# hank-kuo-cs/Volumetric-Primitives-Net

Measured on AMD Instinct MI355X. Metric: render+Chamfer fwd+bwd images/sec, higher is better.
Workload: dtype f32; 1 GPU; C3: B=64/GPU (global 64), K=32 sphere primitives, 256x256 silhouette+depth, n=256 pts/prim (N=8192) vs M=2048 GT points, Chamfer+L1 fwd+bwd; global_batch=64, parallelism=dp1, collective=none, sampling=fresh Philox draws every step (device step counter, 28 steps drawn)

## Files before the change

### volumetric-primitives-net_amd/csrc/sampler.hip

```cpp
#include "vpn_raster_common.h"
#include "vpn_chamfer_feat.h"

namespace vpn {

constexpr int SAMP_BLOCK = 256;

struct PrimLds {
    Pose pose;
    float v[3];
    int cum[7];
    int kind;
};

__device__ inline void cuboid_quota(const float v[3], int n, int cum[7]) {
#pragma clang fp contract(off)
    float w = v[0], h = v[1], d = v[2];
    float hd = h * d, dw = d * w, wh = w * h;
    float total = (hd + dw + wh) * 2.0f;
    float area[6] = {hd, hd, dw, dw, wh, wh};
    int acc = 0;
    cum[0] = 0;
#pragma unroll
    for (int f = 0; f < 5; ++f) {
        float weight = area[f] / total;
        int c = (int)rintf((float)n * weight);
        acc += c;
        cum[f + 1] = acc;
    }
    cum[6] = n;
}

__device__ inline void canonical_coeff(const PrimLds& P, int p, const float u[3], float c[3]) {
    if (P.kind == VPN_SPHERE) {
        const float w0 = 1.0f - 2.0f * u[0];
        const float ce0 = 2.0f * sqrtf(u[0] * (1.0f - u[0]));
        const float w = fmaf(VPN_HALF_PI_EXCESS, ce0, w0);
        const float ce = fmaf(-VPN_HALF_PI_EXCESS, w0, ce0);
        const float azim = u[1] * 2.0f * VPN_PI;
        float sa, ca;
        sincosf(azim, &sa, &ca);
        c[0] = ce * sa;
        c[1] = w;
        c[2] = ce * ca;
    } else {
        c[0] = -1.0f + 2.0f * u[0];
        c[1] = -1.0f + 2.0f * u[1];
        c[2] = -1.0f + 2.0f * u[2];
#pragma unroll
        for (int f = 0; f < 6; ++f) {
            if (p >= P.cum[f] && p < P.cum[f + 1]) c[f >> 1] = (f & 1) ? -1.0f : 1.0f;
        }
    }
}

__device__ inline void load_prim(PrimLds& P, const float* prm, int kind, int n) {
    P.pose = make_pose(prm[3], prm[4], prm[5], prm[6]);
    P.v[0] = prm[0]; P.v[1] = prm[1]; P.v[2] = prm[2];
    P.kind = kind == VPN_SPHERE ? VPN_SPHERE : VPN_CUBOID;
    if (P.kind == VPN_CUBOID) cuboid_quota(P.v, n, P.cum);
}

__device__ inline void load_prim_saved(PrimLds& P, const float* prm, int kind, int n, const float4* rk) {
    const float4 p0 = rk[R_FIN + 3], p1 = rk[R_FIN + 4], p2 = rk[R_FIN + 5], p3 = rk[R_FIN + 6];
    Pose& S = P.pose;
    S.R.m[0][0] = p0.x; S.R.m[0][1] = p0.y; S.R.m[0][2] = p0.z; S.R.m[1][0] = p0.w; S.R.m[1][1] = p1.x; S.R.m[1][2] = p1.y;
    S.R.m[2][0] = p1.z; S.R.m[2][1] = p1.w; S.R.m[2][2] = p2.x; S.x = p2.y; S.y = p2.z; S.z = p2.w;
    S.w = p3.x; S.sh = p3.y; S.ch = p3.z; S.inv_len = p3.w;
    P.v[0] = prm[0]; P.v[1] = prm[1]; P.v[2] = prm[2];
    P.kind = kind == VPN_SPHERE ? VPN_SPHERE : VPN_CUBOID;
    if (P.kind == VPN_CUBOID) cuboid_quota(P.v, n, P.cum);
}

__device__ inline void sample_wg(PrimLds& P, float* red, int b, int k,
    const float* __restrict__ params, const int32_t* __restrict__ kinds, const float* __restrict__ u,
    uint64_t seed, uint64_t sample_base, int K, int n,
    float* __restrict__ points, const RasterPrep& rp, const FeatJob* feat, const FeatJob* gt = nullptr,
    float* red_gt = nullptr) {
    const float* prm = params + ((size_t)b * K + k) * VPN_PARAM_STRIDE;
    if (threadIdx.x == 0) load_prim(P, prm, kinds[k], n);
    if (gt) feat_slice_early(*gt, b, k, 64, red_gt);
    Camera C;
    const bool rec_lane = rp.rec && threadIdx.x == 64;
    if (rec_lane) C = make_camera(rp.cam + b * 3);
    if (rp.zero_me && k == 0) {
        if (b == 0 && threadIdx.x >= 128 && threadIdx.x < 130) rp.zero_me[threadIdx.x - 128] = 0;
        if (b == 0 && threadIdx.x == 130) *reinterpret_cast<uint64_t*>(rp.zero_me + 2) = seed;
        if (threadIdx.x == 131) rp.zero_me[4 + 4 * b + 3] = 0;
    }
    __syncthreads();
    if (gt && threadIdx.x == 65) feat_slice_publish(*gt, b, k, 64, red_gt);
    if (rec_lane) {
        float4 r[R_REC];
        make_record_from(C, P.pose, prm, kinds[k] == VPN_SPHERE ? VPN_SPHERE : VPN_CUBOID, rp.H, rp.W, rp.sigma, r);
        float4* out = rp.rec + ((size_t)b * K + k) * R_REC;
#pragma unroll
        for (int i = 0; i < R_REC; ++i) out[i] = r[i];
    }
    const float tx = prm[7], ty = prm[8], tz = prm[9];
    const float* ub = u ? u + ((size_t)b * K + k) * n * 3 : nullptr;
    float* out = points + ((size_t)b * K + k) * n * 3;
    float nv = 0.0f;
    for (int p = threadIdx.x; p < n; p += SAMP_BLOCK) {
        float uu[3];
        if (ub) { uu[0] = ub[p * 3]; uu[1] = ub[p * 3 + 1]; uu[2] = ub[p * 3 + 2]; }
        else philox_uniform3(seed, sample_base + (uint64_t)b, (uint32_t)k, (uint32_t)p, uu);
        float c[3];
        canonical_coeff(P, p, uu, c);
        float px, py, pz;
        {
#pragma clang fp contract(off)
            const float x = c[0] * P.v[0], y = c[1] * P.v[1], z = c[2] * P.v[2];
            const Mat3& R = P.pose.R;
            px = (R.m[0][0] * x + R.m[0][1] * y + R.m[0][2] * z) + tx;
            py = (R.m[1][0] * x + R.m[1][1] * y + R.m[1][2] * z) + ty;
            pz = (R.m[2][0] * x + R.m[2][1] * y + R.m[2][2] * z) + tz;
        }
        st3(out + p * 3, px, py, pz);
        if (feat) nv = fmaxf(nv, feat_point(*feat, b, k * n + p, px, py, pz));
    }
    if (feat) {
        if (k == K - 1) for (int j = K * n + (int)threadIdx.x; j < feat->Np; j += SAMP_BLOCK) feat_point(*feat, b, j, 0.f, 0.f, 0.f);
        if (feat->tboxes) __threadfence_block();
        feat_finish_slice(*feat, b, k, nv, red);
        feat_tile_boxes(*feat, b, k * n, k == K - 1 ? feat->Np : (k + 1) * n);
    }
}

__global__ __launch_bounds__(SAMP_BLOCK) void sample_fwd_kernel(
    const float* __restrict__ params, const int32_t* __restrict__ kinds, const float* __restrict__ u,
    uint64_t seed, const uint64_t* __restrict__ seed_dev, uint64_t sample_base, int K, int n,
    float* __restrict__ points, const RasterPrep rp) {
    __shared__ PrimLds P;
    if (seed_dev) seed += *seed_dev;
    sample_wg(P, nullptr, blockIdx.y, blockIdx.x, params, kinds, u, seed, sample_base, K, n, points, rp, nullptr);
}

__host__ __device__ inline int rec_workgroups(int BK) { return ((BK + SAMP_BLOCK - 1) / SAMP_BLOCK + 7) & ~7; }
__host__ __device__ inline int ord_workgroups(int B) { return (B + 7) & ~7; }

__global__ __launch_bounds__(SAMP_BLOCK) void sample_feat_fwd_kernel(
    const float* __restrict__ params, const int32_t* __restrict__ kinds, const float* __restrict__ u,
    uint64_t seed, const uint64_t* __restrict__ seed_dev, uint64_t sample_base, int B, int K, int n,
    float* __restrict__ points, const RasterPrep rp, const FeatJob pred, const FeatJob gt) {
    __shared__ PrimLds P;
    __shared__ float red[SAMP_BLOCK / 64];
    static_assert(SAMP_BLOCK == CFEAT_THREADS, "feature slices are written by sampler-sized workgroups");
    if (seed_dev) seed += *seed_dev;
    const int nrec = rp.rec ? rec_workgroups(B * K) : 0;
    if ((int)blockIdx.x < nrec) {
        const int bk = blockIdx.x * SAMP_BLOCK + threadIdx.x;
        if (bk < B * K) {
            const int rb = bk / K, rk = bk - rb * K;
            const float* prm = params + (size_t)bk * VPN_PARAM_STRIDE;
            const Camera C = make_camera(rp.cam + rb * 3);
            const Pose Pq = make_pose(prm[3], prm[4], prm[5], prm[6]);
            float4* out = rp.rec + (size_t)bk * R_REC;
            make_record_put(C, Pq, prm, kinds[rk] == VPN_SPHERE ? VPN_SPHERE : VPN_CUBOID, rp.H, rp.W, rp.sigma,
                            [&](int i, const float4 v) { out[i] = v; });
        }
        return;
    }
    const int nord = gt.perm ? ord_workgroups(B) : 0;
    if ((int)blockIdx.x < nrec + nord) {
        int ob, oy;
        feat_decode((int)blockIdx.x - nrec, nord, ob, oy);
        if (ob < B) feat_order_wg(gt, ob);
        return;
    }
    RasterPrep rq = rp;
    rq.rec = nullptr;
    int b, sy;
    feat_decode((int)blockIdx.x - nrec - nord, B, b, sy);
    __shared__ float red_gt[SAMP_BLOCK / 64];
    sample_wg(P, red, b, sy, params, kinds, u, seed, sample_base, K, n, points, rq, &pred, &gt, red_gt);
}

__global__ __launch_bounds__(SAMP_BLOCK) void sample_bwd_kernel(
    const float* __restrict__ params, const int32_t* __restrict__ kinds, const float* __restrict__ u,
    uint64_t seed, const uint64_t* __restrict__ seed_dev, uint64_t sample_base, int K, int n,
    const float* __restrict__ grad_points, float* __restrict__ grad_params) {
    __shared__ PrimLds P;
    if (seed_dev) seed += *seed_dev;
    __shared__ float red[SAMP_BLOCK / 64][12];
    const int k = blockIdx.x, b = blockIdx.y;
    const float* prm = params + ((size_t)b * K + k) * VPN_PARAM_STRIDE;
    if (threadIdx.x == 0) load_prim(P, prm, kinds[k], n);
    __syncthreads();
    const float* ub = u ? u + ((size_t)b * K + k) * n * 3 : nullptr;
    const float* gp = grad_points + ((size_t)b * K + k) * n * 3;
    float acc[12];
#pragma unroll
    for (int i = 0; i < 12; ++i) acc[i] = 0.0f;
    for (int p = threadIdx.x; p < n; p += SAMP_BLOCK) {
        float uu[3];
        if (ub) { uu[0] = ub[p * 3]; uu[1] = ub[p * 3 + 1]; uu[2] = ub[p * 3 + 2]; }
        else philox_uniform3(seed, sample_base + (uint64_t)b, (uint32_t)k, (uint32_t)p, uu);
        float c[3];
        canonical_coeff(P, p, uu, c);
        float g[3] = {gp[p * 3], gp[p * 3 + 1], gp[p * 3 + 2]};
#pragma unroll
        for (int r = 0; r < 3; ++r) {
#pragma unroll
            for (int a = 0; a < 3; ++a) acc[r * 3 + a] += g[r] * c[a];
            acc[9 + r] += g[r];
        }
    }
    const int lane = threadIdx.x & 63, wave = threadIdx.x >> 6;
#pragma unroll
    for (int i = 0; i < 12; ++i) {
        float s = wave_sum(acc[i]);
        if (lane == 0) red[wave][i] = s;
    }
    __syncthreads();
    if (threadIdx.x == 0) {
        float G[3][3], gt[3];
        for (int r = 0; r < 3; ++r) {
            for (int a = 0; a < 3; ++a) {
                float s = 0.0f;
                for (int w = 0; w < SAMP_BLOCK / 64; ++w) s += red[w][r * 3 + a];
                G[r][a] = s;
            }
            float s = 0.0f;
            for (int w = 0; w < SAMP_BLOCK / 64; ++w) s += red[w][9 + r];
            gt[r] = s;
        }
        const Mat3& R = P.pose.R;
        float gR[3][3], gv[3], gq[4];
        for (int a = 0; a < 3; ++a) {
            gv[a] = R.m[0][a] * G[0][a] + R.m[1][a] * G[1][a] + R.m[2][a] * G[2][a];
            for (int r = 0; r < 3; ++r) gR[r][a] = G[r][a] * P.v[a];
        }
        pose_backward(P.pose, prm[3], prm[4], prm[5], gR, gq);
        float* o = grad_params + ((size_t)b * K + k) * VPN_PARAM_STRIDE;
        o[0] = gv[0]; o[1] = gv[1]; o[2] = gv[2];
        o[3] = gq[0]; o[4] = gq[1]; o[5] = gq[2]; o[6] = gq[3];
        o[7] = gt[0]; o[8] = gt[1]; o[9] = gt[2];
    }
}

#ifndef SCB_BLOCK
#define SCB_BLOCK 128
#endif
struct StepExtras {
    const float* emd_dist = nullptr; const int32_t* emd_assign = nullptr; float emd_coef = 0.f;
    const float* dv_dist1 = nullptr; const int32_t* dv_idx1 = nullptr;
    const float* dv_dist2 = nullptr; const int32_t* dv_idx2 = nullptr;
    float dv_c1 = 0.f, dv_c2 = 0.f;
    const float* cn_points = nullptr; const float* cn_gt = nullptr; const float* cn_mat = nullptr;
    const float* cn_dist1 = nullptr; const int32_t* cn_idx1 = nullptr; const float* cn_dist2 = nullptr; const int32_t* cn_idx2 = nullptr;
    float cn_c1 = 0.f, cn_c2 = 0.f; int cn_M = 0;
};

template <bool EXTRAS>
__global__ __launch_bounds__(SCB_BLOCK) void sample_chamfer_bwd_kernel(
    const float* __restrict__ params, const int32_t* __restrict__ kinds, const float* __restrict__ u,
    uint64_t seed, const uint64_t* __restrict__ seed_dev, uint64_t sample_base, int K, int n,
    const float* __restrict__ points, const float* __restrict__ gt, int M, const float* __restrict__ dist1, const int32_t* __restrict__ idx1,
    const float* __restrict__ dist2, const int32_t* __restrict__ idx2, const float* __restrict__ grad_loss_b,
    float w1, float w2, float* __restrict__ grad_params, const RasterFinish rf, const StepExtras ex) {
    __shared__ PrimLds P;
    __shared__ float red[SCB_BLOCK / 64][12];
    __shared__ float fin[SCB_BLOCK / 64][12];
    __shared__ float rgrad[10];
    if (seed_dev) seed += *seed_dev;
    const int k = blockIdx.x, b = blockIdx.y, N = K * n;
    const float* prm = params + ((size_t)b * K + k) * VPN_PARAM_STRIDE;
    if (threadIdx.x == 0) {
        if (rf.rec) load_prim_saved(P, prm, kinds[k], n, rf.rec + ((size_t)b * K + k) * R_REC);
        else load_prim(P, prm, kinds[k], n);
    }
    if (rf.partial) {
        float fv[16];
        raster_finish_gather(b * K + k, K, rf.ntile, rf.words, rf.masks, rf.partial, (int)(threadIdx.x >> 6) * 64, SCB_BLOCK, fv);
        const float tot = wave_reduce16_swap(fv);
        if ((threadIdx.x & 3) == 0 && (threadIdx.x & 63) < 48) fin[threadIdx.x >> 6][(threadIdx.x & 63) >> 2] = tot;
    }
    __syncthreads();
    const float* ub = u ? u + ((size_t)b * K + k) * n * 3 : nullptr;
    const float* A = points + (size_t)b * N * 3;
    const float* G2 = gt + (size_t)b * M * 3;
    const float gl = grad_loss_b ? grad_loss_b[b] : rf.scale[0];
    const float ca = gl * w1 / (float)N, cb = gl * w2 / (float)M;
    float acc[12];
#pragma unroll
    for (int i = 0; i < 12; ++i) acc[i] = 0.0f;
    const float tx = prm[7], ty = prm[8], tz = prm[9];
    const float vmin = fminf(fminf(fabsf(P.v[0]), fabsf(P.v[1])), fabsf(P.v[2]));
    const float big = fmaxf(fmaxf(fmaxf(fabsf(tx), fabsf(ty)), fabsf(tz)), fmaxf(fmaxf(fabsf(P.v[0]), fabsf(P.v[1])), fabsf(P.v[2])));
    const bool recover = vmin >= 1.0e-2f * big && vmin > 1e-20f;
    const float iv0 = recover ? 1.0f / P.v[0] : 0.0f, iv1 = recover ? 1.0f / P.v[1] : 0.0f, iv2 = recover ? 1.0f / P.v[2] : 0.0f;
    auto add = [&](int pl, float gx, float gy, float gz) {
        float c[3];
        if (recover) {
            const int i = k * n + pl;
            const F3 a = ld3(A + i * 3);
            const float dx = a.x - tx, dy = a.y - ty, dz = a.z - tz;
            const Mat3& R = P.pose.R;
            c[0] = (R.m[0][0] * dx + R.m[1][0] * dy + R.m[2][0] * dz) * iv0;
            c[1] = (R.m[0][1] * dx + R.m[1][1] * dy + R.m[2][1] * dz) * iv1;
            c[2] = (R.m[0][2] * dx + R.m[1][2] * dy + R.m[2][2] * dz) * iv2;
        } else {
            float uu[3];
            if (ub) { uu[0] = ub[pl * 3]; uu[1] = ub[pl * 3 + 1]; uu[2] = ub[pl * 3 + 2]; }
            else philox_uniform3(seed, sample_base + (uint64_t)b, (uint32_t)k, (uint32_t)pl, uu);
            canonical_coeff(P, pl, uu, c);
        }
        const float g[3] = {gx, gy, gz};
#pragma unroll
        for (int r = 0; r < 3; ++r) {
#pragma unroll
            for (int a = 0; a < 3; ++a) acc[r * 3 + a] += g[r] * c[a];
            acc[9 + r] += g[r];
        }
    };
    const bool cn_on = EXTRAS && ex.cn_points;
    const float* Sm = ex.cn_mat + b * 9;
    const float S0 = cn_on ? Sm[0] : 0.f, S1 = cn_on ? Sm[1] : 0.f, S2 = cn_on ? Sm[2] : 0.f, S3 = cn_on ? Sm[3] : 0.f, S4 = cn_on ? Sm[4] : 0.f,
                S5 = cn_on ? Sm[5] : 0.f, S6 = cn_on ? Sm[6] : 0.f, S7 = cn_on ? Sm[7] : 0.f, S8 = cn_on ? Sm[8] : 0.f;
    auto add_canon = [&](int pl, float gx, float gy, float gz) {
        add(pl, S0 * gx + S3 * gy + S6 * gz, S1 * gx + S4 * gy + S7 * gz, S2 * gx + S5 * gy + S8 * gz);
    };
    for (int pl = threadIdx.x; pl < n; pl += SCB_BLOCK) {
        const int i = k * n + pl, j = idx1[(size_t)b * N + i];
        const float coef = ca / dist1[(size_t)b * N + i];
        const F3 a = ld3(A + i * 3), g = ld3(G2 + j * 3);
        float gx = coef * (a.x - g.x), gy = coef * (a.y - g.y), gz = coef * (a.z - g.z);
        if (EXTRAS && ex.emd_dist) {
// ... 277 lines not shown
                float s = 0.0f;
                for (int w = 0; w < MESH_BLOCK / 64; ++w) s += red[w][r * 3 + a];
                G[r][a] = s;
            }
            float s = 0.0f;
            for (int w = 0; w < MESH_BLOCK / 64; ++w) s += red[w][9 + r];
            gt[r] = s;
        }
        const Mat3& R = S.R;
        float gR[3][3], gv[3], gq[4];
        for (int a = 0; a < 3; ++a) {
            gv[a] = R.m[0][a] * G[0][a] + R.m[1][a] * G[1][a] + R.m[2][a] * G[2][a];
            for (int r = 0; r < 3; ++r) gR[r][a] = G[r][a] * prm[a];
        }
        pose_backward(S, prm[3], prm[4], prm[5], gR, gq);
        float* og = grad_params + ((size_t)b * K + k) * VPN_PARAM_STRIDE;
        og[0] = gv[0]; og[1] = gv[1]; og[2] = gv[2];
        og[3] = gq[0]; og[4] = gq[1]; og[5] = gq[2]; og[6] = gq[3];
        og[7] = gt[0]; og[8] = gt[1]; og[9] = gt[2];
    }
}

__device__ inline Mat3 mat_mul(const Mat3& A, const Mat3& B) {
    Mat3 C;
#pragma unroll
    for (int i = 0; i < 3; ++i)
#pragma unroll
        for (int j = 0; j < 3; ++j) C.m[i][j] = A.m[i][0] * B.m[0][j] + A.m[i][1] * B.m[1][j] + A.m[i][2] * B.m[2][j];
    return C;
}

__device__ inline Mat3 camera_matrix(float elev, float azim, float angle, int to_object) {
    const float e = elev / 360.0f, a = azim / 360.0f;
    const Mat3 Re = make_pose(0.0f, 0.0f, -1.0f, e).R;
    const float yx = Re.m[0][1], yy = Re.m[1][1], yz = Re.m[2][1];
    if (to_object) {
        const Mat3 Rx = make_pose(1.0f, 0.0f, 0.0f, -angle / 360.0f).R;
        const Mat3 Ra = make_pose(yx, yy, yz, -a).R;
        const Mat3 Rb = make_pose(0.0f, 0.0f, -1.0f, -e).R;
        return mat_mul(Rb, mat_mul(Ra, Rx));
    }
    const Mat3 Ra = make_pose(yx, yy, yz, a).R;
    return mat_mul(Ra, Re);
}

__global__ __launch_bounds__(TR_BLOCK) void camera_transform_kernel(
    const float* __restrict__ pts, const float* __restrict__ dists, const float* __restrict__ elevs,
    const float* __restrict__ azims, const float* __restrict__ angles, int N, int to_object, int transpose,
    float* __restrict__ out) {
    __shared__ Mat3 S;
    const int b = blockIdx.y;
    if (threadIdx.x == 0) {
        Mat3 M = camera_matrix(elevs[b], azims[b], angles ? angles[b] : 0.0f, to_object);
        if (transpose) {
            Mat3 T;
            for (int i = 0; i < 3; ++i) for (int j = 0; j < 3; ++j) T.m[i][j] = M.m[j][i];
            M = T;
        }
        S = M;
    }
    __syncthreads();
    const Mat3& R = S;
    const float d = dists[b];
    for (int p = blockIdx.x * TR_BLOCK + threadIdx.x; p < N; p += gridDim.x * TR_BLOCK) {
        const float* pp = pts + ((size_t)b * N + p) * 3;
        const float x = pp[0], y = pp[1], z = pp[2];
        float ox = R.m[0][0] * x + R.m[0][1] * y + R.m[0][2] * z;
        float oy = R.m[1][0] * x + R.m[1][1] * y + R.m[1][2] * z;
        float oz = R.m[2][0] * x + R.m[2][1] * y + R.m[2][2] * z;
        if (to_object) { ox *= d; oy *= d; oz *= d; }
        else { ox /= d; oy /= d; oz /= d; }
        float* o = out + ((size_t)b * N + p) * 3;
        o[0] = ox; o[1] = oy; o[2] = oz;
    }
}

__global__ __launch_bounds__(64) void camera_matrix_kernel(const float* __restrict__ dists, const float* __restrict__ elevs,
                                                          const float* __restrict__ azims, const float* __restrict__ angles,
                                                          int B, int to_object, float* __restrict__ mat) {
    const int b = blockIdx.x * 64 + threadIdx.x;
    if (b >= B) return;
    const Mat3 M = camera_matrix(elevs[b], azims[b], angles ? angles[b] : 0.0f, to_object);
    const float d = dists[b];
    for (int i = 0; i < 3; ++i) for (int j = 0; j < 3; ++j) mat[b * 9 + i * 3 + j] = to_object ? M.m[i][j] * d : M.m[i][j] / d;
}

__global__ __launch_bounds__(256) void raster_prep_kernel(const float* __restrict__ params,
                                                          const int32_t* __restrict__ kinds,
                                                          const float* __restrict__ cam, int BK, int K, int H, int W,
                                                          float sigma, float4* __restrict__ rec, int* __restrict__ zero_me) {
    const int bk = blockIdx.x * 256 + threadIdx.x;
    if (zero_me && bk < 4) zero_me[bk] = 0;
    if (bk >= BK) return;
    const int b = bk / K, k = bk - b * K;
    if (zero_me && k == 0) zero_me[4 + 4 * b + 3] = 0;
    float4 r[R_REC];
    make_record(params + (size_t)bk * VPN_PARAM_STRIDE, kinds[k] == VPN_SPHERE ? VPN_SPHERE : VPN_CUBOID, cam, b, H, W, sigma, r);
    float4* out = rec + (size_t)bk * R_REC;
#pragma unroll
    for (int i = 0; i < R_REC; ++i) out[i] = r[i];
}


int launch_raster_prep(const float* params, const int32_t* kinds, const float* cam, int B, int K, int H, int W,
                       float sigma, void* records, int* zero_me, hipStream_t s) {
    const int BK = B * K;
    VPN_LAUNCH(raster_prep_kernel, dim3((BK + 255) / 256), dim3(256), 0, s, params, kinds, cam, BK, K, H, W, sigma,
               (float4*)records, zero_me);
    VPN_LAUNCH_CHECK();
    return 0;
}

}

using namespace vpn;

static int launch_sample_fwd(const float* params, const int32_t* kinds, const float* u, uint64_t seed,
                             const uint64_t* seed_dev, uint64_t sample_base, int B, int K, int n, float* points,
                             const RasterPrep& rp, void* stream) {
    if (!params || !kinds || !points) return VPN_E_BADARG;
    if (B <= 0 || K <= 0 || n <= 0) return VPN_E_BADARG;
    if (B > 65535) return VPN_E_TOOBIG;
    VPN_LAUNCH(sample_fwd_kernel, dim3(K, B), dim3(SAMP_BLOCK), 0, (hipStream_t)stream, params, kinds, u,
                       seed, seed_dev, sample_base, K, n, points, rp);
    VPN_LAUNCH_CHECK();
    return 0;
}

extern "C" int vpn_sample_fwd(const float* params, const int32_t* kinds, const float* u, uint64_t seed,
                              const uint64_t* seed_dev, uint64_t sample_base, int B, int K, int n, float* points,
                              void* stream) {
    return launch_sample_fwd(params, kinds, u, seed, seed_dev, sample_base, B, K, n, points, RasterPrep{}, stream);
}

extern "C" int vpn_hotpath_sample_fwd(const float* params, const int32_t* kinds, const float* u, uint64_t seed,
                                      const uint64_t* seed_dev, uint64_t sample_base, int B, int K, int n, float* points,
                                      const float* cam, int H, int W, float sigma, void* records, void* loss_ws,
                                      const float* gt_points, int M, void* chamfer_ws, size_t chamfer_ws_bytes,
                                      void* stream) {
    if (!cam || !records || H <= 0 || W <= 0 || !(sigma > 0.f) || K > VPN_MAX_PRIMS) return VPN_E_BADARG;
    if (((uintptr_t)records & 15) != 0) return VPN_E_BADARG;
    RasterPrep rp;
    rp.cam = cam; rp.H = H; rp.W = W; rp.sigma = sigma; rp.rec = (float4*)records; rp.zero_me = (int*)loss_ws;
    if (!chamfer_ws) return launch_sample_fwd(params, kinds, u, seed, seed_dev, sample_base, B, K, n, points, rp, stream);
    if (!params || !kinds || !points || !gt_points) return VPN_E_BADARG;
    if (B <= 0 || K <= 0 || n <= 0 || M <= 0 || K > CFEAT_SLOTS) return VPN_E_BADARG;
    if ((long long)B * K * n > 0x7fffffffLL) return VPN_E_TOOBIG;
    FeatJob pred, gt;
    int rc = chamfer_feat_jobs(chamfer_ws, chamfer_ws_bytes, B, K * n, M, points, gt_points, &pred, &gt);
    if (rc) return rc;
    pred.ysplit = K;
    gt.ysplit = K;
    const unsigned nrec = (unsigned)rec_workgroups(B * K) + (gt.perm ? (unsigned)ord_workgroups(B) : 0u);
    VPN_LAUNCH(sample_feat_fwd_kernel, dim3((unsigned)B * (unsigned)K + nrec), dim3(SAMP_BLOCK), 0, (hipStream_t)stream,
               params, kinds, u, seed, seed_dev, sample_base, B, K, n, points, rp, pred, gt);
    VPN_LAUNCH_CHECK();
    return 0;
}

extern "C" int vpn_hotpath_fused_features(int B, int K, int n, int M) {
    if (B <= 0 || K <= 0 || n <= 0 || M <= 0 || K > CFEAT_SLOTS) return 0;
    FeatJob a, b;
    static float dummy[4] __attribute__((aligned(16)));
    return chamfer_feat_jobs(dummy, (size_t)-1, B, K * n, M, nullptr, nullptr, &a, &b) == 0 ? 1 : 0;
}

extern "C" int vpn_sample_bwd(const float* params, const int32_t* kinds, const float* u, uint64_t seed,
                              const uint64_t* seed_dev, uint64_t sample_base, int B, int K, int n, const float* grad_points,
                              float* grad_params, void* stream) {
    if (!params || !kinds || !grad_points || !grad_params) return VPN_E_BADARG;
    if (B <= 0 || K <= 0 || n <= 0) return VPN_E_BADARG;
    if (B > 65535) return VPN_E_TOOBIG;
    VPN_LAUNCH(sample_bwd_kernel, dim3(K, B), dim3(SAMP_BLOCK), 0, (hipStream_t)stream, params, kinds, u,
                       seed, seed_dev, sample_base, K, n, grad_points, grad_params);
    VPN_LAUNCH_CHECK();
    return 0;
}

extern "C" int vpn_transform_fwd(const float* points, const float* q, const float* t, int B, int N, float* out,
                                 void* stream) {
    if (!points || !q || !out) return VPN_E_BADARG;
    if (B <= 0 || N <= 0) return VPN_E_BADARG;
    if (B > 65535) return VPN_E_TOOBIG;
    int gx = (N + TR_BLOCK - 1) / TR_BLOCK;
    if (gx > 1024) gx = 1024;
    VPN_LAUNCH(transform_fwd_kernel, dim3(gx, B), dim3(TR_BLOCK), 0, (hipStream_t)stream, points, q, t, N,
                       out);
    VPN_LAUNCH_CHECK();
    return 0;
}

extern "C" int vpn_transform_bwd(const float* points, const float* q, const float* grad_out, int B, int N,
                                 float* grad_points, float* grad_q, float* grad_t, void* stream) {
    if (!points || !q || !grad_out) return VPN_E_BADARG;
    if (B <= 0 || N <= 0) return VPN_E_BADARG;
    VPN_LAUNCH(transform_bwd_kernel, dim3(B), dim3(TR_BLOCK), 0, (hipStream_t)stream, points, q, grad_out,
                       N, grad_points, grad_q, grad_t);
    VPN_LAUNCH_CHECK();
    return 0;
}

static int camera_launch(const float* points, const float* dists, const float* elevs, const float* azims,
                         const float* angles, int B, int N, int to_object, int transpose, float* out, void* stream) {
    if (!points || !dists || !elevs || !azims || !out) return VPN_E_BADARG;
    if (to_object && !angles) return VPN_E_BADARG;
    if (B <= 0 || N <= 0) return VPN_E_BADARG;
    if (B > 65535) return VPN_E_TOOBIG;
    int gx = (N + TR_BLOCK - 1) / TR_BLOCK;
    if (gx > 1024) gx = 1024;
    VPN_LAUNCH(camera_transform_kernel, dim3(gx, B), dim3(TR_BLOCK), 0, (hipStream_t)stream, points, dists, elevs,
               azims, angles, N, to_object, transpose, out);
    VPN_LAUNCH_CHECK();
    return 0;
}

extern "C" int vpn_camera_matrix(const float* dists, const float* elevs, const float* azims, const float* angles, int B,
                                 int to_object, float* mat, void* stream) {
    if (!dists || !elevs || !azims || !mat || (to_object && !angles) || B <= 0) return VPN_E_BADARG;
    VPN_LAUNCH(camera_matrix_kernel, dim3((B + 63) / 64), dim3(64), 0, (hipStream_t)stream, dists, elevs, azims, angles, B, to_object, mat);
    VPN_LAUNCH_CHECK();
    return 0;
}

extern "C" int vpn_camera_transform_fwd(const float* points, const float* dists, const float* elevs,
                                        const float* azims, const float* angles, int B, int N, int to_object,
                                        float* out, void* stream) {
    return camera_launch(points, dists, elevs, azims, angles, B, N, to_object, 0, out, stream);
}

extern "C" int vpn_camera_transform_bwd(const float* grad_out, const float* dists, const float* elevs,
                                        const float* azims, const float* angles, int B, int N, int to_object,
                                        float* grad_points, void* stream) {
    return camera_launch(grad_out, dists, elevs, azims, angles, B, N, to_object, 1, grad_points, stream);
}

static constexpr size_t SCB_MAX_LDS = 60 * 1024;
static constexpr size_t scb_match_lds(int M) {
    return (size_t)((M + SCB_BLOCK - 1) / SCB_BLOCK) * 64 * (SCB_BLOCK / 64) * sizeof(int2);
}
static_assert(scb_match_lds(VPN_FUSED_BWD_MAX_GT) <= SCB_MAX_LDS && scb_match_lds(VPN_FUSED_BWD_MAX_GT + 1) > SCB_MAX_LDS,
              "VPN_FUSED_BWD_MAX_GT is the largest M whose match lists fit");

static int launch_scb(const float* params, const int32_t* kinds, const float* u, uint64_t seed,
                      const uint64_t* seed_dev, uint64_t sample_base, int B, int K, int n, const float* points,
                      const float* gt_points, int M, const float* dist1, const int32_t* idx1,
                      const float* dist2, const int32_t* idx2, const float* grad_loss_b, float w1,
                      float w2, float* grad_params, const RasterFinish& rf, void* stream, const StepExtras* ex = nullptr) {
    if (!params || !kinds || !points || !gt_points || !dist1 || !idx1 || !dist2 || !idx2 || !grad_params)
        return VPN_E_BADARG;
    if (!grad_loss_b && !rf.scale) return VPN_E_BADARG;
    if (B <= 0 || K <= 0 || n <= 0 || M <= 0) return VPN_E_BADARG;
    if (B > 65535 || (long long)K * n > 0x7fffffffLL / 3) return VPN_E_TOOBIG;
    constexpr int BLK = SCB_BLOCK;
    const size_t lds = scb_match_lds(M);
    if (lds > SCB_MAX_LDS) return VPN_E_TOOBIG;
    if (ex)
        VPN_LAUNCH_AS("sample_chamfer_bwd_kernel<step>", sample_chamfer_bwd_kernel<true>, dim3(K, B), dim3(BLK), lds, (hipStream_t)stream, params, kinds, u, seed,
                      seed_dev, sample_base, K, n, points, gt_points, M, dist1, idx1, dist2, idx2, grad_loss_b, w1, w2, grad_params, rf, *ex);
    else
        VPN_LAUNCH_AS("sample_chamfer_bwd_kernel", sample_chamfer_bwd_kernel<false>, dim3(K, B), dim3(BLK), lds, (hipStream_t)stream, params, kinds, u, seed,
                      seed_dev, sample_base, K, n, points, gt_points, M, dist1, idx1, dist2, idx2, grad_loss_b, w1, w2, grad_params, rf, StepExtras{});
    VPN_LAUNCH_CHECK();
    return 0;
}

extern "C" int vpn_sample_chamfer_bwd(const float* params, const int32_t* kinds, const float* u, uint64_t seed,
                                      const uint64_t* seed_dev, uint64_t sample_base, int B, int K, int n, const float* points,
                                      const float* gt_points, int M, const float* dist1, const int32_t* idx1,
                                      const float* dist2, const int32_t* idx2, const float* grad_loss_b, float w1,
                                      float w2, float* grad_params, void* stream) {
    return launch_scb(params, kinds, u, seed, seed_dev, sample_base, B, K, n, points, gt_points, M, dist1, idx1, dist2, idx2,
                      grad_loss_b, w1, w2, grad_params, RasterFinish{}, stream);
}

extern "C" int vpn_hotpath_bwd(const float* params, const int32_t* kinds, const float* u, uint64_t seed,
                               const uint64_t* seed_dev, uint64_t sample_base, int B, int K, int n, const float* points,
                               const float* gt_points, int M, const float* dist1, const int32_t* idx1,
                               const float* dist2, const int32_t* idx2, const float* grad_loss_b, float w1, float w2,
                               const float* cam, int H, int W, const void* records, const void* workspace,
                               const float* grad_total, float* grad_params, void* stream) {
    if (!cam || !records || !workspace || H <= 0 || W <= 0) return VPN_E_BADARG;
    RasterFinish rf;
    rf.rec = (const float4*)records;
    rf.ntile = ((W + R_TW - 1) / R_TW) * ((H + R_TH - 1) / R_TH);
    rf.words = (K + 63) / 64;
    rf.masks = reinterpret_cast<const unsigned long long*>(reinterpret_cast<const char*>(records) + (size_t)B * K * R_REC * sizeof(float4));
    rf.partial = (const float*)workspace;
    rf.scale = grad_total;
    return launch_scb(params, kinds, u, seed, seed_dev, sample_base, B, K, n, points, gt_points, M, dist1, idx1, dist2, idx2,
                      grad_loss_b, w1, w2, grad_params, rf, stream);
}

extern "C" int vpn_trainstep_bwd(const float* params, const int32_t* kinds, uint64_t seed, const uint64_t* seed_dev,
                                 uint64_t sample_base, int B, int K, int n, const float* points, const float* gt_points, int M,
                                 const float* dist1, const int32_t* idx1, const float* dist2, const int32_t* idx2,
                                 float w1, float w2, const float* cam, int H, int W, const void* records,
                                 const void* workspace, const float* grad_total,
                                 const float* emd_dist, const int32_t* emd_assign, float emd_coef,
                                 const float* dv_dist1, const int32_t* dv_idx1, const float* dv_dist2, const int32_t* dv_idx2,
                                 float dv_c1, float dv_c2,
                                 const float* cn_points, const float* cn_gt, const float* cn_mat, const float* cn_dist1,
                                 const int32_t* cn_idx1, const float* cn_dist2, const int32_t* cn_idx2, float cn_c1, float cn_c2,
                                 int cn_M, float* grad_params, void* stream) {
    if (!grad_total) return VPN_E_BADARG;
    if (emd_dist && (!emd_assign || K * n != M)) return VPN_E_BADARG;
    if (dv_dist1 && (!dv_idx1 || !dv_dist2 || !dv_idx2)) return VPN_E_BADARG;
    if (cn_points && (!cn_gt || !cn_mat || !cn_dist1 || !cn_idx1 || !cn_dist2 || !cn_idx2 || cn_M <= 0)) return VPN_E_BADARG;
    RasterFinish rf;
// ... 50 lines not shown
```

### volumetric-primitives-net_amd/csrc/vpn_chamfer_feat.h

```cpp
#pragma once
#include "vpn_common.h"

namespace vpn {

constexpr int CM_ROWB = 48;
__device__ inline void split3_bf16(float x, unsigned short p[3]) {
#pragma clang fp contract(off)
    const unsigned u0 = __float_as_uint(x);
    p[0] = (unsigned short)(u0 >> 16);
    const float r1 = x - __uint_as_float(u0 & 0xFFFF0000u);
    const unsigned u1 = __float_as_uint(r1);
    p[1] = (unsigned short)(u1 >> 16);
    const float r2 = r1 - __uint_as_float(u1 & 0xFFFF0000u);
    p[2] = (unsigned short)(__float_as_uint(r2) >> 16);
}

constexpr float CM_S16 = 2048.0f;
constexpr int CM_ROWB16 = 32;
__device__ inline void split2_f16(float X, _Float16 h[2]) {
    h[0] = (_Float16)X;
    h[1] = (_Float16)(X - (float)h[0]);
}

struct Row16 { uint4 lo, hi; };
__device__ inline Row16 make_row16(float x, float y, float z, float n) {
#pragma clang fp contract(off)
    _Float16 hx[2], hy[2], hz[2], pn[3];
    split2_f16(CM_S16 * x, hx); split2_f16(CM_S16 * y, hy); split2_f16(CM_S16 * z, hz);
    if (n < 1.0e30f) {
        const float ns = (CM_S16 * CM_S16) * n;
        pn[0] = (_Float16)(ns * 3.0517578125e-05f);
        const float r1 = ns - (float)pn[0] * 32768.0f;
        pn[1] = (_Float16)(r1 * 0.0625f);
        pn[2] = (_Float16)(r1 - (float)pn[1] * 16.0f);
    } else {
        pn[0] = (_Float16)65504.0f; pn[1] = (_Float16)0.0f; pn[2] = (_Float16)0.0f;
    }
    auto bits = [](_Float16 v) { return (unsigned)__builtin_bit_cast(unsigned short, v); };
    auto pk = [&](_Float16 lo, _Float16 hi) { return bits(lo) | (bits(hi) << 16); };
    const _Float16 zero = (_Float16)0.0f;
    return Row16{make_uint4(pk(hx[0], hx[0]), pk(hx[1], hy[0]), pk(hy[0], hy[1]), pk(hz[0], hz[0])),
                 make_uint4(pk(hz[1], pn[0]), pk(pn[1], pn[2]), pk(zero, zero), pk(zero, zero))};
}
__device__ inline Row16 sentinel_row16() { return make_row16(0.0f, 0.0f, 0.0f, 3.0e38f); }
__device__ inline void write_row16(unsigned short* H, size_t row, float x, float y, float z, float n) {
    const Row16 r = make_row16(x, y, z, n);
    uint4* dst = reinterpret_cast<uint4*>(reinterpret_cast<unsigned char*>(H) + row * CM_ROWB16);
    dst[0] = r.lo; dst[1] = r.hi;
}

__device__ inline void write_row(unsigned short* H, size_t row, float x, float y, float z, float n) {
#pragma clang fp contract(off)
    unsigned short px[3], py[3], pz[3], pn[3];
    split3_bf16(x, px); split3_bf16(y, py); split3_bf16(z, pz); split3_bf16(n, pn);
    auto pk = [](unsigned short lo, unsigned short hi) { return (unsigned)lo | ((unsigned)hi << 16); };
    uint4* dst = reinterpret_cast<uint4*>(reinterpret_cast<unsigned char*>(H) + row * CM_ROWB);
    dst[0] = make_uint4(pk(px[0], px[0]), pk(px[1], px[0]), pk(px[2], px[1]), pk(py[0], py[0]));
    dst[1] = make_uint4(pk(py[1], py[0]), pk(py[2], py[1]), pk(pz[0], pz[0]), pk(pz[1], pz[0]));
    dst[2] = make_uint4(pk(pz[2], pz[1]), pk(pn[0], pn[1]), pk(pn[2], 0), 0u);
}


constexpr int CFEAT_THREADS = 256;
#ifndef CFEAT_WGPTS
#define CFEAT_WGPTS 256
#endif
constexpr int CFEAT_SLOTS = 64;
constexpr int CFEAT_PTS = 4;

struct FeatJob {
    const float* pts; int N, Np, ysplit;
    float* F; unsigned int* nmax; unsigned short* H;
    int rows16;
    float* tboxes;
    int32_t* perm;
};

__device__ inline void feat_decode(int id, int B, int& b, int& sy) {
    const int per = B >> 3;
    if ((B & 7) == 0) { const int xcd = id & 7, r = id >> 3; b = xcd * per + r % per; sy = r / per; }
    else { b = id % B; sy = id / B; }
}

__device__ inline float feat_wave_max(float v) {
#define VPN_FDPP(v, ctrl, rmask) \
    __int_as_float(__builtin_amdgcn_update_dpp(__float_as_int(v), __float_as_int(v), ctrl, rmask, 0xf, false))
    v = fmaxf(v, VPN_FDPP(v, 0x111, 0xf)); v = fmaxf(v, VPN_FDPP(v, 0x112, 0xf));
    v = fmaxf(v, VPN_FDPP(v, 0x114, 0xf)); v = fmaxf(v, VPN_FDPP(v, 0x118, 0xf));
    v = fmaxf(v, VPN_FDPP(v, 0x142, 0xa)); v = fmaxf(v, VPN_FDPP(v, 0x143, 0xc));
#undef VPN_FDPP
    return __int_as_float(__builtin_amdgcn_readlane(__float_as_int(v), 63));
}

__device__ inline float feat_point(const FeatJob& J, int b, int j, float x, float y, float z) {
#pragma clang fp contract(off)
    float* f = J.F + (size_t)b * 4 * J.Np;
    float n = 3.0e38f, nv = 0.0f;
    if (j < J.N) { n = x * x + y * y + z * z; nv = n; } else { x = 0.f; y = 0.f; z = 0.f; }
    f[j] = x; f[J.Np + j] = y; f[2 * J.Np + j] = z; f[3 * J.Np + j] = n;
    if (J.H) {
        if (J.rows16) write_row16(J.H, (size_t)b * J.Np + j, x, y, z, n);
        else write_row(J.H, (size_t)b * J.Np + j, x, y, z, n);
    }
    return nv;
}

__device__ inline void feat_finish_slice(const FeatJob& J, int b, int by, float nv, float* red) {
    if (by == 0 && (int)threadIdx.x >= J.ysplit && threadIdx.x < CFEAT_SLOTS) J.nmax[b * CFEAT_SLOTS + threadIdx.x] = 0u;
    nv = feat_wave_max(nv);
    if ((threadIdx.x & 63) == 0) red[threadIdx.x >> 6] = nv;
    __syncthreads();
    if (threadIdx.x == 0) {
        float m = red[0];
        for (int w = 1; w < CFEAT_THREADS / 64; ++w) m = fmaxf(m, red[w]);
        J.nmax[b * CFEAT_SLOTS + by] = __float_as_uint(m);
    }
}

template <bool MAX>
__device__ inline float feat_wave_minmax(float v) {
#define VPN_FDPP(v, ctrl, rmask) \
    __int_as_float(__builtin_amdgcn_update_dpp(__float_as_int(v), __float_as_int(v), ctrl, rmask, 0xf, false))
#define VPN_FOP(a, b) (MAX ? fmaxf(a, b) : fminf(a, b))
    v = VPN_FOP(v, VPN_FDPP(v, 0x111, 0xf)); v = VPN_FOP(v, VPN_FDPP(v, 0x112, 0xf));
    v = VPN_FOP(v, VPN_FDPP(v, 0x114, 0xf)); v = VPN_FOP(v, VPN_FDPP(v, 0x118, 0xf));
    v = VPN_FOP(v, VPN_FDPP(v, 0x142, 0xa)); v = VPN_FOP(v, VPN_FDPP(v, 0x143, 0xc));
#undef VPN_FOP
#undef VPN_FDPP
    return __int_as_float(__builtin_amdgcn_readlane(__float_as_int(v), 63));
}

constexpr int CFEAT_TILE = 256;
constexpr int CFEAT_BOXF = 8;
constexpr int CSKIP_MIN_TARGETS = 4096;
constexpr int CORD_MAX = 2048;
constexpr int CCAND_CAP = 512;
constexpr int CCAND_MAX_TARGETS = 65535;
constexpr int CCAND_CELL = 16;

__device__ inline float* feat_tile_box(float* boxes, int Np, int b, int t) {
    return boxes + ((size_t)b * (Np >> 5) + t) * CFEAT_BOXF;
}

__device__ inline void feat_tile_boxes(const FeatJob& J, int b, int rlo, int rhi) {
    if (!J.tboxes || rlo >= rhi) return;
    const float* f = J.F + (size_t)b * 4 * J.Np;
    const int lane = threadIdx.x & 63, wave = threadIdx.x >> 6;
    const float inf = __builtin_inff();
    for (int t = rlo / CFEAT_TILE + wave; t * CFEAT_TILE < rhi; t += CFEAT_THREADS / 64) {
        const int r0 = t * CFEAT_TILE, r1 = min(r0 + CFEAT_TILE, J.Np);
        float lo[3] = {-inf, -inf, -inf}, hi[3] = {inf, inf, inf};
        if (r0 >= rlo && r1 <= rhi) {
            lo[0] = lo[1] = lo[2] = inf; hi[0] = hi[1] = hi[2] = -inf;
            const int rn = min(r1, J.N);
            for (int r = r0 + lane; r < rn; r += 64) {
                const float x = f[r], y = f[J.Np + r], z = f[2 * J.Np + r];
                lo[0] = fminf(lo[0], x); hi[0] = fmaxf(hi[0], x);
                lo[1] = fminf(lo[1], y); hi[1] = fmaxf(hi[1], y);
                lo[2] = fminf(lo[2], z); hi[2] = fmaxf(hi[2], z);
            }
#pragma unroll
            for (int a = 0; a < 3; ++a) { lo[a] = feat_wave_minmax<false>(lo[a]); hi[a] = feat_wave_minmax<true>(hi[a]); }
        }
        if (lane == 0) {
            float4* o = reinterpret_cast<float4*>(feat_tile_box(J.tboxes, J.Np, b, t));
            o[0] = make_float4(lo[0], lo[1], lo[2], hi[0]);
            o[1] = make_float4(hi[1], hi[2], 0.f, 0.f);
        }
    }
}

__device__ inline void feat_order_wg(const FeatJob& J, int b) {
    constexpr int CORD_PER = CORD_MAX / CFEAT_THREADS;
    __shared__ unsigned short cnt[CORD_MAX / 64][64];
    __shared__ float bred[6][CFEAT_THREADS / 64];
    __shared__ int cbase[64];
    const int N = J.N, tid = threadIdx.x, lane = tid & 63, wave = tid >> 6;
    const float* p = J.pts + (size_t)b * N * 3;
    int32_t* po = J.perm + (size_t)b * J.Np;
    if (N > CORD_MAX) {
        for (int i = tid; i < N; i += CFEAT_THREADS) po[i] = i;
        return;
    }
    const float inf = __builtin_inff();
    float lo[3] = {inf, inf, inf}, hi[3] = {-inf, -inf, -inf};
#pragma unroll 2
    for (int j = 0; j < CORD_PER; ++j) {
        const F3 v = ld3(p + min(tid + j * CFEAT_THREADS, N - 1) * 3);
        lo[0] = fminf(lo[0], v.x); hi[0] = fmaxf(hi[0], v.x);
        lo[1] = fminf(lo[1], v.y); hi[1] = fmaxf(hi[1], v.y);
        lo[2] = fminf(lo[2], v.z); hi[2] = fmaxf(hi[2], v.z);
    }
#pragma unroll
    for (int a = 0; a < 3; ++a) {
        const float l = feat_wave_minmax<false>(lo[a]), h = feat_wave_minmax<true>(hi[a]);
        if (lane == 0) { bred[a][wave] = l; bred[3 + a][wave] = h; }
    }
    const int nch = (N + 63) >> 6;
    for (int e = tid; e < nch * 64; e += CFEAT_THREADS) cnt[e >> 6][e & 63] = 0;
    __syncthreads();
    float o3[3], sc[3];
#pragma unroll
    for (int a = 0; a < 3; ++a) {
        float l = bred[a][0], h = bred[3 + a][0];
        for (int w = 1; w < CFEAT_THREADS / 64; ++w) { l = fminf(l, bred[a][w]); h = fmaxf(h, bred[3 + a][w]); }
        o3[a] = l;
        sc[a] = h > l ? 4.0f / (h - l) : 0.0f;
    }
    static_assert(CORD_PER * 6 <= 64, "the cells of a lane's points are packed into 64 bits");
    unsigned long long keys = 0;
#pragma unroll 2
    for (int j = 0; j < CORD_PER; ++j) {
        const F3 v = ld3(p + min(tid + j * CFEAT_THREADS, N - 1) * 3);
        const float c[3] = {v.x, v.y, v.z};
        unsigned k = 0;
#pragma unroll
        for (int a = 0; a < 3; ++a) {
            const unsigned ca = (unsigned)(int)fminf(fmaxf((c[a] - o3[a]) * sc[a], 0.0f), 3.0f);
            k |= ((ca & 1u) << a) | ((ca >> 1) << (a + 3));
        }
        keys |= (unsigned long long)k << (6 * j);
    }
    auto rank_of = [&](unsigned k, bool ok, int& rank, int& count) {
        unsigned long long eq = __ballot(ok);
#pragma unroll
        for (int bit = 0; bit < 6; ++bit) {
            const bool s = (k >> bit) & 1u;
            const unsigned long long m = __ballot(s);
            eq &= s ? m : ~m;
        }
        rank = __popcll(eq & ((1ull << lane) - 1ull));
        count = __popcll(eq);
    };
#pragma unroll 2
    for (int j = 0; j < CORD_PER; ++j) {
        const int c = wave + j * (CFEAT_THREADS / 64);
        if (c >= nch) break;
        const bool ok = tid + j * CFEAT_THREADS < N;
        const unsigned k = (unsigned)(keys >> (6 * j)) & 63u;
        int rank, count;
        rank_of(k, ok, rank, count);
        if (ok && rank == 0) cnt[c][k] = (unsigned short)count;
    }
    __syncthreads();
    if (tid < 64) {
        int s = 0;
#pragma unroll 8
        for (int c = 0; c < nch; ++c) { const int t = cnt[c][tid]; cnt[c][tid] = (unsigned short)s; s += t; }
        int inc = s;
#pragma unroll
        for (int o = 1; o < 64; o <<= 1) { const int t2 = __shfl_up(inc, o, 64); if (lane >= o) inc += t2; }
        cbase[tid] = inc - s;
    }
    __syncthreads();
#pragma unroll 2
    for (int j = 0; j < CORD_PER; ++j) {
        const int c = wave + j * (CFEAT_THREADS / 64);
        if (c >= nch) break;
        const int i = tid + j * CFEAT_THREADS;
        const bool ok = i < N;
        const unsigned k = (unsigned)(keys >> (6 * j)) & 63u;
        int rank, count;
        rank_of(k, ok, rank, count);
        if (ok) po[cbase[k] + cnt[c][k] + rank] = i;
    }
}

__device__ inline void feat_slice(const FeatJob& J, int b, int by, float* red) {
    const float* pb = J.pts + (size_t)b * J.N * 3;
    float nv = 0.f;
    const int per = ((J.Np + J.ysplit - 1) / J.ysplit + 63) & ~63;
    const int jlo = by * per, jhi = min(J.Np, jlo + per);
    for (int j0p = jlo + threadIdx.x; j0p < jhi; j0p += CFEAT_PTS * CFEAT_THREADS) {
        float xs[CFEAT_PTS], ys[CFEAT_PTS], zs[CFEAT_PTS];
#pragma unroll
        for (int u = 0; u < CFEAT_PTS; ++u) {
            const int j = min(j0p + u * CFEAT_THREADS, J.N - 1);
            const F3 v3 = ld3(pb + j * 3);
            xs[u] = v3.x; ys[u] = v3.y; zs[u] = v3.z;
        }
#pragma unroll
        for (int u = 0; u < CFEAT_PTS; ++u) {
            const int j = j0p + u * CFEAT_THREADS;
            if (j >= jhi) break;
            nv = fmaxf(nv, feat_point(J, b, j, xs[u], ys[u], zs[u]));
        }
    }
    if (J.tboxes) __threadfence_block();
    feat_finish_slice(J, b, by, nv, red);
    feat_tile_boxes(J, b, jlo, jhi);
}

__device__ inline void feat_slice_early(const FeatJob& J, int b, int by, int first, float* red) {
    if (by == 0 && (int)threadIdx.x >= J.ysplit && threadIdx.x < CFEAT_SLOTS) J.nmax[b * CFEAT_SLOTS + threadIdx.x] = 0u;
    if ((int)threadIdx.x < first) return;
    const float* pb = J.pts + (size_t)b * J.N * 3;
    float nv = 0.f;
    const int per = ((J.Np + J.ysplit - 1) / J.ysplit + 63) & ~63;
    const int jlo = by * per, jhi = min(J.Np, jlo + per), lanes = CFEAT_THREADS - first;
    for (int j = jlo + (int)threadIdx.x - first; j < jhi; j += lanes) {
        const F3 v3 = ld3(pb + min(j, J.N - 1) * 3);
        nv = fmaxf(nv, feat_point(J, b, j, v3.x, v3.y, v3.z));
    }
    nv = feat_wave_max(nv);
    if ((threadIdx.x & 63) == 0) red[threadIdx.x >> 6] = nv;
}
__device__ inline void feat_slice_publish(const FeatJob& J, int b, int by, int first, const float* red) {
    float m = red[first >> 6];
    for (int w = (first >> 6) + 1; w < CFEAT_THREADS / 64; ++w) m = fmaxf(m, red[w]);
    J.nmax[b * CFEAT_SLOTS + by] = __float_as_uint(m);
}

int chamfer_feat_jobs(void* workspace, size_t workspace_bytes, int B, int N, int M, const float* p1, const float* p2,
                      FeatJob* job1, FeatJob* job2);
int chamfer_wgsums(const void* workspace, size_t workspace_bytes, int B, int N, int M, const float** sums1, int* g1,
                   const float** sums2, int* g2);

}
```

Baseline: 459,700 images/s.

## Map one primitive per wavefront in fused sampler+feature forward kernel

Adds a wave-per-primitive path to the fused sampling/feature forward kernel for n<=256: each 64-lane wave handles one primitive, keeping pose and quota in scalar registers instead of LDS and dropping the workgroup barriers. Each lane processes several points per iteration, and tile bounding boxes are reduced in registers as points are produced rather than re-read from global memory. The GT feature slice is also computed per wave. This trades per-block LDS sharing and barriers for more wave-level work, and changes the grid shape to B*ceil(K/4) blocks.

```diff
diff --git a/volumetric-primitives-net_amd/csrc/sampler.hip b/volumetric-primitives-net_amd/csrc/sampler.hip
--- a/volumetric-primitives-net_amd/csrc/sampler.hip
+++ b/volumetric-primitives-net_amd/csrc/sampler.hip
@@ -71,6 +71,16 @@
     if (P.kind == VPN_CUBOID) cuboid_quota(P.v, n, P.cum);
 }
 
+__device__ inline void prim_point(const PrimLds& P, const float c[3], float tx, float ty, float tz,
+                                  float& px, float& py, float& pz) {
+#pragma clang fp contract(off)
+    const float x = c[0] * P.v[0], y = c[1] * P.v[1], z = c[2] * P.v[2];
+    const Mat3& R = P.pose.R;
+    px = (R.m[0][0] * x + R.m[0][1] * y + R.m[0][2] * z) + tx;
+    py = (R.m[1][0] * x + R.m[1][1] * y + R.m[1][2] * z) + ty;
+    pz = (R.m[2][0] * x + R.m[2][1] * y + R.m[2][2] * z) + tz;
+}
+
 __device__ inline void sample_wg(PrimLds& P, float* red, int b, int k,
     const float* __restrict__ params, const int32_t* __restrict__ kinds, const float* __restrict__ u,
     uint64_t seed, uint64_t sample_base, int K, int n,
@@ -107,14 +117,7 @@
         float c[3];
         canonical_coeff(P, p, uu, c);
         float px, py, pz;
-        {
-#pragma clang fp contract(off)
-            const float x = c[0] * P.v[0], y = c[1] * P.v[1], z = c[2] * P.v[2];
-            const Mat3& R = P.pose.R;
-            px = (R.m[0][0] * x + R.m[0][1] * y + R.m[0][2] * z) + tx;
-            py = (R.m[1][0] * x + R.m[1][1] * y + R.m[1][2] * z) + ty;
-            pz = (R.m[2][0] * x + R.m[2][1] * y + R.m[2][2] * z) + tz;
-        }
+        prim_point(P, c, tx, ty, tz, px, py, pz);
         st3(out + p * 3, px, py, pz);
         if (feat) nv = fmaxf(nv, feat_point(*feat, b, k * n + p, px, py, pz));
     }
@@ -123,6 +126,116 @@
         if (feat->tboxes) __threadfence_block();
         feat_finish_slice(*feat, b, k, nv, red);
         feat_tile_boxes(*feat, b, k * n, k == K - 1 ? feat->Np : (k + 1) * n);
+    }
+}
+
+constexpr int SAMP_WAVE_MAX_N = 256;
+#ifndef SAMP_WAVE_PTS
+#define SAMP_WAVE_PTS 4
+#endif
+
+__device__ inline float wave_uniform(float v) { return __int_as_float(__builtin_amdgcn_readfirstlane(__float_as_int(v))); }
+
+template <int W>
+__device__ inline float sample_wave_group(const PrimLds& P, float tx, float ty, float tz, int b, int k, int p0, int n,
+                                          const float* __restrict__ ub, uint64_t seed, uint64_t gb, float* __restrict__ out,
+                                          const FeatJob& feat, float lo[3], float hi[3]) {
+    const int pl = p0 + (int)(threadIdx.x & 63);
+    float uu[W][3], c[W][3];
+    if (ub) {
+#pragma unroll
+        for (int j = 0; j < W; ++j) {
+            const F3 v = ld3(ub + min(pl + 64 * j, n - 1) * 3);
+            uu[j][0] = v.x; uu[j][1] = v.y; uu[j][2] = v.z;
+        }
+    } else {
+#pragma unroll
+        for (int j = 0; j < W; ++j) philox_uniform3(seed, gb, (uint32_t)k, (uint32_t)(pl + 64 * j), uu[j]);
+    }
+    if (P.kind == VPN_SPHERE) {
+#pragma unroll
+        for (int j = 0; j < W; ++j) canonical_coeff(P, pl + 64 * j, uu[j], c[j]);
+    } else {
+#pragma unroll
+        for (int j = 0; j < W; ++j) canonical_coeff(P, pl + 64 * j, uu[j], c[j]);
+    }
+    float nv = 0.0f;
+#pragma unroll
+    for (int j = 0; j < W; ++j) {
+        const int p = pl + 64 * j;
+        float px, py, pz;
+        prim_point(P, c[j], tx, ty, tz, px, py, pz);
+        if (p < n) {
+            st3(out + p * 3, px, py, pz);
+            nv = fmaxf(nv, feat_point(feat, b, k * n + p, px, py, pz));
+            lo[0] = fminf(lo[0], px); hi[0] = fmaxf(hi[0], px);
+            lo[1] = fminf(lo[1], py); hi[1] = fmaxf(hi[1], py);
+            lo[2] = fminf(lo[2], pz); hi[2] = fmaxf(hi[2], pz);
+        }
+    }
+    return nv;
+}
+
+__device__ inline void sample_wave(int b, int k, const float* __restrict__ params, const int32_t* __restrict__ kinds,
+                                   const float* __restrict__ u, uint64_t seed, uint64_t sample_base, int K, int n,
+                                   float* __restrict__ points, int* __restrict__ zero_me, const FeatJob& pred, const FeatJob& gt) {
+    const int lane = threadIdx.x & 63;
+    const FeatSliceHead gh = feat_slice_wave_begin(gt, b, k);
+    if (zero_me && k == 0) {
+        if (b == 0 && lane < 2) zero_me[lane] = 0;
+        if (b == 0 && lane == 2) *reinterpret_cast<uint64_t*>(zero_me + 2) = seed;
+        if (lane == 3) zero_me[4 + 4 * b + 3] = 0;
+    }
+    if (k == 0 && lane >= pred.ysplit) pred.nmax[b * CFEAT_SLOTS + lane] = 0u;
+    const float* prm = params + ((size_t)b * K + k) * VPN_PARAM_STRIDE;
+    PrimLds P;
+    load_prim(P, prm, kinds[k], n);
+#pragma unroll
+    for (int i = 0; i < 3; ++i) {
+#pragma unroll
+        for (int j = 0; j < 3; ++j) P.pose.R.m[i][j] = wave_uniform(P.pose.R.m[i][j]);
+        P.v[i] = wave_uniform(P.v[i]);
+    }
+    if (P.kind == VPN_CUBOID) {
+#pragma unroll
+        for (int f = 0; f < 7; ++f) P.cum[f] = __builtin_amdgcn_readfirstlane(P.cum[f]);
+    }
+    const float tx = prm[7], ty = prm[8], tz = prm[9];
+    feat_slice_wave_end(gt, b, k, gh);
+    const float* ub = u ? u + ((size_t)b * K + k) * n * 3 : nullptr;
+    float* out = points + ((size_t)b * K + k) * n * 3;
+    const uint64_t gb = sample_base + (uint64_t)b;
+    const bool regbox = pred.tboxes && n % CFEAT_TILE == 0;
+    static_assert(CFEAT_TILE % (64 * SAMP_WAVE_PTS) == 0, "whole groups of the wave make up a tile of the scan");
+    const float inf = __builtin_inff();
+    float nv = 0.0f;
+    float lo[3] = {inf, inf, inf}, hi[3] = {-inf, -inf, -inf};
+#pragma unroll 1
+    for (int p0 = 0; p0 < n; p0 += 64 * SAMP_WAVE_PTS) {
+        const int live = (n - p0 + 63) >> 6;
+        if (live >= SAMP_WAVE_PTS) {
+            nv = fmaxf(nv, sample_wave_group<SAMP_WAVE_PTS>(P, tx, ty, tz, b, k, p0, n, ub, seed, gb, out, pred, lo, hi));
+        } else {
+            for (int j = 0; j < live; ++j)
+                nv = fmaxf(nv, sample_wave_group<1>(P, tx, ty, tz, b, k, p0 + 64 * j, n, ub, seed, gb, out, pred, lo, hi));
+        }
+        if (regbox && (p0 + 64 * SAMP_WAVE_PTS) % CFEAT_TILE == 0) {
+            float blo[3], bhi[3];
+#pragma unroll
+            for (int a = 0; a < 3; ++a) {
+                blo[a] = feat_wave_minmax<false>(lo[a]); bhi[a] = feat_wave_minmax<true>(hi[a]);
+                lo[a] = inf; hi[a] = -inf;
+            }
+            if (lane == 0) feat_put_box(pred, b, (k * n + p0) / CFEAT_TILE, blo, bhi);
+        }
+    }
+    if (k == K - 1) for (int j = K * n + lane; j < pred.Np; j += 64) feat_point(pred, b, j, 0.f, 0.f, 0.f);
+    nv = feat_wave_max(nv);
+    if (lane == 0) pred.nmax[b * CFEAT_SLOTS + k] = __float_as_uint(nv);
+    if (pred.tboxes && !regbox) {
+        __builtin_amdgcn_fence(__ATOMIC_SEQ_CST, "wavefront");
+        __builtin_amdgcn_s_waitcnt(0x0F70);
+        feat_tile_boxes_by(pred, b, k * n, k == K - 1 ? pred.Np : (k + 1) * n, 0, 1);
     }
 }
 
@@ -138,12 +251,11 @@
 __host__ __device__ inline int rec_workgroups(int BK) { return ((BK + SAMP_BLOCK - 1) / SAMP_BLOCK + 7) & ~7; }
 __host__ __device__ inline int ord_workgroups(int B) { return (B + 7) & ~7; }
 
+template <bool WAVE>
 __global__ __launch_bounds__(SAMP_BLOCK) void sample_feat_fwd_kernel(
     const float* __restrict__ params, const int32_t* __restrict__ kinds, const float* __restrict__ u,
     uint64_t seed, const uint64_t* __restrict__ seed_dev, uint64_t sample_base, int B, int K, int n,
     float* __restrict__ points, const RasterPrep rp, const FeatJob pred, const FeatJob gt) {
-    __shared__ PrimLds P;
-    __shared__ float red[SAMP_BLOCK / 64];
     static_assert(SAMP_BLOCK == CFEAT_THREADS, "feature slices are written by sampler-sized workgroups");
     if (seed_dev) seed += *seed_dev;
     const int nrec = rp.rec ? rec_workgroups(B * K) : 0;
@@ -167,12 +279,20 @@
         if (ob < B) feat_order_wg(gt, ob);
         return;
     }
-    RasterPrep rq = rp;
-    rq.rec = nullptr;
     int b, sy;
     feat_decode((int)blockIdx.x - nrec - nord, B, b, sy);
-    __shared__ float red_gt[SAMP_BLOCK / 64];
-    sample_wg(P, red, b, sy, params, kinds, u, seed, sample_base, K, n, points, rq, &pred, &gt, red_gt);
+    if constexpr (WAVE) {
+        const int k = sy * (SAMP_BLOCK / 64) + __builtin_amdgcn_readfirstlane((int)(threadIdx.x >> 6));
+        if (k >= K) return;
+        sample_wave(b, k, params, kinds, u, seed, sample_base, K, n, points, rp.zero_me, pred, gt);
+    } else {
+        __shared__ PrimLds P;
+        __shared__ float red[SAMP_BLOCK / 64];
+        __shared__ float red_gt[SAMP_BLOCK / 64];
+        RasterPrep rq = rp;
+        rq.rec = nullptr;
+        sample_wg(P, red, b, sy, params, kinds, u, seed, sample_base, K, n, points, rq, &pred, &gt, red_gt);
+    }
 }
 
 __global__ __launch_bounds__(SAMP_BLOCK) void sample_bwd_kernel(
@@ -756,8 +876,14 @@
     pred.ysplit = K;
     gt.ysplit = K;
     const unsigned nrec = (unsigned)rec_workgroups(B * K) + (gt.perm ? (unsigned)ord_workgroups(B) : 0u);
-    VPN_LAUNCH(sample_feat_fwd_kernel, dim3((unsigned)B * (unsigned)K + nrec), dim3(SAMP_BLOCK), 0, (hipStream_t)stream,
-               params, kinds, u, seed, seed_dev, sample_base, B, K, n, points, rp, pred, gt);
+    if (n <= SAMP_WAVE_MAX_N)
+        VPN_LAUNCH_AS("sample_feat_fwd_kernel", sample_feat_fwd_kernel<true>,
+                      dim3((unsigned)B * (unsigned)((K + SAMP_BLOCK / 64 - 1) / (SAMP_BLOCK / 64)) + nrec), dim3(SAMP_BLOCK), 0,
+                      (hipStream_t)stream, params, kinds, u, seed, seed_dev, sample_base, B, K, n, points, rp, pred, gt);
+    else
+        VPN_LAUNCH_AS("sample_feat_fwd_kernel", sample_feat_fwd_kernel<false>, dim3((unsigned)B * (unsigned)K + nrec),
+                      dim3(SAMP_BLOCK), 0, (hipStream_t)stream, params, kinds, u, seed, seed_dev, sample_base, B, K, n,
+                      points, rp, pred, gt);
     VPN_LAUNCH_CHECK();
     return 0;
 }
diff --git a/volumetric-primitives-net_amd/csrc/vpn_chamfer_feat.h b/volumetric-primitives-net_amd/csrc/vpn_chamfer_feat.h
--- a/volumetric-primitives-net_amd/csrc/vpn_chamfer_feat.h
+++ b/volumetric-primitives-net_amd/csrc/vpn_chamfer_feat.h
@@ -142,12 +142,18 @@
     return boxes + ((size_t)b * (Np >> 5) + t) * CFEAT_BOXF;
 }
 
-__device__ inline void feat_tile_boxes(const FeatJob& J, int b, int rlo, int rhi) {
+__device__ inline void feat_put_box(const FeatJob& J, int b, int t, const float lo[3], const float hi[3]) {
+    float4* o = reinterpret_cast<float4*>(feat_tile_box(J.tboxes, J.Np, b, t));
+    o[0] = make_float4(lo[0], lo[1], lo[2], hi[0]);
+    o[1] = make_float4(hi[1], hi[2], 0.f, 0.f);
+}
+
+__device__ inline void feat_tile_boxes_by(const FeatJob& J, int b, int rlo, int rhi, int wave, int nwaves) {
     if (!J.tboxes || rlo >= rhi) return;
     const float* f = J.F + (size_t)b * 4 * J.Np;
-    const int lane = threadIdx.x & 63, wave = threadIdx.x >> 6;
+    const int lane = threadIdx.x & 63;
     const float inf = __builtin_inff();
-    for (int t = rlo / CFEAT_TILE + wave; t * CFEAT_TILE < rhi; t += CFEAT_THREADS / 64) {
+    for (int t = rlo / CFEAT_TILE + wave; t * CFEAT_TILE < rhi; t += nwaves) {
         const int r0 = t * CFEAT_TILE, r1 = min(r0 + CFEAT_TILE, J.Np);
         float lo[3] = {-inf, -inf, -inf}, hi[3] = {inf, inf, inf};
         if (r0 >= rlo && r1 <= rhi) {
@@ -162,12 +168,11 @@
 #pragma unroll
             for (int a = 0; a < 3; ++a) { lo[a] = feat_wave_minmax<false>(lo[a]); hi[a] = feat_wave_minmax<true>(hi[a]); }
         }
-        if (lane == 0) {
-            float4* o = reinterpret_cast<float4*>(feat_tile_box(J.tboxes, J.Np, b, t));
-            o[0] = make_float4(lo[0], lo[1], lo[2], hi[0]);
-            o[1] = make_float4(hi[1], hi[2], 0.f, 0.f);
-        }
-    }
+        if (lane == 0) feat_put_box(J, b, t, lo, hi);
+    }
+}
+__device__ inline void feat_tile_boxes(const FeatJob& J, int b, int rlo, int rhi) {
+    feat_tile_boxes_by(J, b, rlo, rhi, threadIdx.x >> 6, CFEAT_THREADS / 64);
 }
 
 __device__ inline void feat_order_wg(const FeatJob& J, int b) {
@@ -311,6 +316,30 @@
     J.nmax[b * CFEAT_SLOTS + by] = __float_as_uint(m);
 }
 
+struct FeatSliceHead { F3 v; int j, jhi; };
+__device__ inline FeatSliceHead feat_slice_wave_begin(const FeatJob& J, int b, int by) {
+    const int per = ((J.Np + J.ysplit - 1) / J.ysplit + 63) & ~63;
+    FeatSliceHead h;
+    h.j = by * per + (int)(threadIdx.x & 63);
+    h.jhi = min(J.Np, by * per + per);
+    h.v = F3{0.f, 0.f, 0.f};
+    if (h.j < h.jhi) h.v = ld3(J.pts + ((size_t)b * J.N + min(h.j, J.N - 1)) * 3);
+    return h;
+}
+__device__ inline void feat_slice_wave_end(const FeatJob& J, int b, int by, const FeatSliceHead& h) {
+    const int lane = threadIdx.x & 63;
+    if (by == 0 && lane >= J.ysplit) J.nmax[b * CFEAT_SLOTS + lane] = 0u;
+    const float* pb = J.pts + (size_t)b * J.N * 3;
+    float nv = 0.f;
+    if (h.j < h.jhi) nv = feat_point(J, b, h.j, h.v.x, h.v.y, h.v.z);
+    for (int j = h.j + 64; j < h.jhi; j += 64) {
+        const F3 v3 = ld3(pb + min(j, J.N - 1) * 3);
+        nv = fmaxf(nv, feat_point(J, b, j, v3.x, v3.y, v3.z));
+    }
+    nv = feat_wave_max(nv);
+    if (lane == 0) J.nmax[b * CFEAT_SLOTS + by] = __float_as_uint(nv);
+}
+
 int chamfer_feat_jobs(void* workspace, size_t workspace_bytes, int B, int N, int M, const float* p1, const float* p2,
                       FeatJob* job1, FeatJob* job2);
 int chamfer_wgsums(const void* workspace, size_t workspace_bytes, int B, int N, int M, const float** sums1, int* g1,
```

New measurement: 461,300 images/s (median of 6 runs). Within noise of the previous version (+0.4%).
